# aanna0701/face-recognition-pytorch

Measured on AMD Instinct MI355X. Metric: train imgs/sec IR-50-layout ResNet50 + ArcFace/PartialFC head, 112x112, higher is better.
Workload: dtype bf16

## Files before the change

### face-recognition-pytorch_amd/frhip/csrc/misc.hip

```cpp
#include <stdarg.h>
#include <stdio.h>
#include <atomic>
#include "common.h"
#include "frhip.h"

namespace frhip {

static thread_local char g_err[512] = "";

void set_error(const char* fmt, ...) {
    va_list ap;
    va_start(ap, fmt);
    vsnprintf(g_err, sizeof(g_err), fmt, ap);
    va_end(ap);
}

int check_launch(const char* what) {
    hipError_t e = hipGetLastError();
    if (e != hipSuccess) {
        set_error("%s: launch failed: %s", what, hipGetErrorString(e));
        return FRHIP_ELAUNCH;
    }
    return FRHIP_OK;
}

int set_dynamic_lds(const void* fn, int bytes, const char* who) {
    constexpr int SLOTS = 256;
    static std::atomic<const void*> fns[SLOTS];
    static std::atomic<uint64_t> devs[SLOTS];
    int dev = 0;
    if (hipGetDevice(&dev) != hipSuccess) { (void)hipGetLastError(); dev = -1; }
    const uint64_t bit = (dev >= 0 && dev < 64) ? 1ull << dev : 0;
    int slot = -1;
    const size_t h = (size_t)(((uintptr_t)fn >> 4) * 0x9E3779B97F4A7C15ull >> 32);
    for (int i = 0; i < SLOTS && slot < 0; ++i) {
        const int s = (int)((h + i) % SLOTS);
        const void* cur = nullptr;
        if (fns[s].compare_exchange_strong(cur, fn) || cur == fn) slot = s;
    }
    if (slot >= 0 && bit && (devs[slot].load() & bit)) return FRHIP_OK;
    if (hipFuncSetAttribute(fn, hipFuncAttributeMaxDynamicSharedMemorySize, bytes) != hipSuccess) {
        set_error("%s: cannot raise dynamic LDS to %d bytes", who, bytes);
        return FRHIP_ELAUNCH;
    }
    if (slot >= 0) devs[slot].fetch_or(bit);
    return FRHIP_OK;
}

int device_cu_count() {
    static std::atomic<int> cus[16];
    int dev = 0;
    if (hipGetDevice(&dev) != hipSuccess || dev < 0 || dev >= 16) { (void)hipGetLastError(); return 256; }
    int v = cus[dev].load();
    if (!v) {
        if (hipDeviceGetAttribute(&v, hipDeviceAttributeMultiprocessorCount, dev) != hipSuccess || v <= 0) v = 256;
        cus[dev].store(v);
    }
    return v;
}

template <typename T>
__global__ void pack_wt_kernel(const float* __restrict__ w, T* __restrict__ wt, int K, int RS, int C) {
    __shared__ float tile[32][33];
    const int rs = blockIdx.z, c0 = blockIdx.x * 32, k0 = blockIdx.y * 32;
    for (int j = threadIdx.y; j < 32; j += blockDim.y) {
        const int k = k0 + j, c = c0 + threadIdx.x;
        tile[j][threadIdx.x] = (k < K && c < C) ? w[((size_t)k * RS + rs) * C + c] : 0.f;
    }
    __syncthreads();
    for (int j = threadIdx.y; j < 32; j += blockDim.y) {
        const int c = c0 + j, k = k0 + threadIdx.x;
        if (c < C && k < K) wt[((size_t)c * RS + rs) * K + k] = from_f32<T>(tile[threadIdx.x][j]);
    }
}

template <typename T>
__global__ void prep_weights_kernel(const frhip_wprep* __restrict__ tab, int ntensors) {
    __shared__ float tile[32][33];
    int lo = 0, hi = ntensors - 1;
    while (lo < hi) {
        const int mid = (lo + hi + 1) >> 1;
        if (tab[mid].tile_begin <= (int)blockIdx.x) lo = mid; else hi = mid - 1;
    }
    const frhip_wprep e = tab[lo];
    const int K = e.k, RS = e.rs, C = e.c;
    const int ct = (C + 31) >> 5, kt = (K + 31) >> 5;
    int t = (int)blockIdx.x - e.tile_begin;
    const int cti = t % ct; t /= ct;
    const int kti = t % kt; const int rs = t / kt;
    const int c0 = cti * 32, k0 = kti * 32;
    const float* __restrict__ w = e.w;
    T* __restrict__ wc = reinterpret_cast<T*>(e.wc);
    T* __restrict__ wt = reinterpret_cast<T*>(e.wt);
    for (int j = threadIdx.y; j < 32; j += blockDim.y) {
        const int k = k0 + j, c = c0 + threadIdx.x;
        float v = 0.f;
        if (k < K && c < C) {
            const size_t idx = ((size_t)k * RS + rs) * C + c;
            v = w[idx];
            if (wc) wc[idx] = from_f32<T>(v);
        }
        tile[j][threadIdx.x] = v;
    }
    __syncthreads();
    if (wt)
        for (int j = threadIdx.y; j < 32; j += blockDim.y) {
            const int c = c0 + j, k = k0 + threadIdx.x;
            if (c < C && k < K) wt[((size_t)c * RS + rs) * K + k] = from_f32<T>(tile[threadIdx.x][j]);
        }
}

template <typename TI, typename TO>
__global__ void transpose2d_kernel(const TI* __restrict__ in, TO* __restrict__ out, int rows, int cols, int ld_out) {
    __shared__ float tile[32][33];
    const int c0 = blockIdx.x * 32, r0 = blockIdx.y * 32;
    for (int j = threadIdx.y; j < 32; j += blockDim.y) {
        const int r = r0 + j, c = c0 + threadIdx.x;
        tile[j][threadIdx.x] = (r < rows && c < cols) ? to_f32<TI>(in[(size_t)r * cols + c]) : 0.f;
    }
    __syncthreads();
    for (int j = threadIdx.y; j < 32; j += blockDim.y) {
        const int c = c0 + j, r = r0 + threadIdx.x;
        if (c < cols && r < ld_out) out[(size_t)c * ld_out + r] = from_f32<TO>(tile[threadIdx.x][j]);
    }
}

template <typename T>
__global__ void pack_stem_kernel(const float* __restrict__ w, T* __restrict__ wp, int K, int kin, int kp) {
    const int i = blockIdx.x * blockDim.x + threadIdx.x;
    if (i >= K * kp) return;
    const int k = i / kp, j = i - k * kp;
    wp[i] = from_f32<T>(j < kin ? w[k * kin + j] : 0.f);
}
__global__ void unpack_stem_grad_kernel(const float* __restrict__ dwp, float* __restrict__ dw, int K, int kin, int kp) {
    const int i = blockIdx.x * blockDim.x + threadIdx.x;
    if (i >= K * kin) return;
    const int k = i / kin, j = i - k * kin;
    dw[i] += dwp[k * kp + j];
}

template <typename T>
__global__ __launch_bounds__(256) void fc_permute_kernel(const float* __restrict__ w, T* __restrict__ wp, int C, int HW) {
    extern __shared__ float sh[];
    const int n = blockIdx.x, c0 = blockIdx.y * 64;
    const size_t row = (size_t)n * C * HW;
    for (int i = threadIdx.x; i < 64 * HW; i += 256) sh[i] = w[row + (size_t)c0 * HW + i];
    __syncthreads();
    for (int i = threadIdx.x; i < 64 * HW; i += 256) {
        const int p = i / 64, c = i - p * 64;
        wp[row + (size_t)p * C + c0 + c] = from_f32<T>(sh[c * HW + p]);
    }
}
__global__ __launch_bounds__(256) void fc_unpermute_grad_kernel(const float* __restrict__ dwp, float* __restrict__ dw, int C, int HW) {
    extern __shared__ float sh[];
    const int n = blockIdx.x, c0 = blockIdx.y * 64;
    const size_t row = (size_t)n * C * HW;
    for (int i = threadIdx.x; i < 64 * HW; i += 256) {
        const int p = i / 64, c = i - p * 64;
        sh[i] = dwp[row + (size_t)p * C + c0 + c];
    }
    __syncthreads();
    for (int i = threadIdx.x; i < 64 * HW; i += 256) {
        const int c = i / HW, p = i - c * HW;
        dw[row + (size_t)c0 * HW + i] += sh[p * 64 + c];
    }
}

__global__ void gather_rows_kernel(const float* __restrict__ src, const int64_t* __restrict__ index,
                                   float* __restrict__ dst, int n, int D) {
    const int vpr = D / 4;
    for (size_t t = (size_t)blockIdx.x * blockDim.x + threadIdx.x; t < (size_t)n * vpr; t += (size_t)gridDim.x * blockDim.x) {
        const int i = (int)(t / vpr), v = (int)(t - (size_t)i * vpr);
        reinterpret_cast<f32x4_t*>(dst)[t] = reinterpret_cast<const f32x4_t*>(src)[(size_t)index[i] * vpr + v];
    }
}
__global__ void scatter_rows_kernel(const float* __restrict__ src, const int64_t* __restrict__ index,
                                    float* __restrict__ dst, int n, int D) {
    const int vpr = D / 4;
    for (size_t t = (size_t)blockIdx.x * blockDim.x + threadIdx.x; t < (size_t)n * vpr; t += (size_t)gridDim.x * blockDim.x) {
        const int i = (int)(t / vpr), v = (int)(t - (size_t)i * vpr);
        reinterpret_cast<f32x4_t*>(dst)[(size_t)index[i] * vpr + v] = reinterpret_cast<const f32x4_t*>(src)[t];
    }
}

}

using namespace frhip;

extern "C" const char* frhip_last_error(void) { return g_err; }
extern "C" int frhip_abi_version(void) { return 1; }

extern "C" int frhip_pack_wt(int dtype, const float* w, void* wt, int k, int rs, int c, hipStream_t stream) {
    return by_dtype(dtype, "frhip_pack_wt", [&](auto t) {
        typedef decltype(t) T;
        dim3 grid((c + 31) / 32, (k + 31) / 32, rs), block(32, 8);
        hipLaunchKernelGGL(pack_wt_kernel<T>, grid, block, 0, stream, w, (T*)wt, k, rs, c);
        return check_launch("frhip_pack_wt");
    });
}

extern "C" int frhip_prep_conv_weights(int dtype, const frhip_wprep* table, int ntensors, int ntiles, hipStream_t stream) {
    return by_dtype(dtype, "frhip_prep_conv_weights", [&](auto t) {
        typedef decltype(t) T;
        if (!table || ntensors < 1 || ntiles < 1) { set_error("frhip_prep_conv_weights: empty table"); return FRHIP_EINVAL; }
        dim3 block(32, 8);
        hipLaunchKernelGGL(prep_weights_kernel<T>, dim3(ntiles), block, 0, stream, table, ntensors);
        return check_launch("frhip_prep_conv_weights");
    });
}

extern "C" int frhip_transpose2d(int dtype_in, int dtype_out, const void* in, void* out, int rows, int cols, int ld_out, hipStream_t stream) {
    if (ld_out < rows) { set_error("frhip_transpose2d: ld_out %d < rows %d", ld_out, rows); return FRHIP_EINVAL; }
    dim3 grid((cols + 31) / 32, (ld_out + 31) / 32), block(32, 8);
    const int key = dtype_in * 2 + dtype_out;
    switch (key) {
        case 0: hipLaunchKernelGGL((transpose2d_kernel<bf16_t, bf16_t>), grid, block, 0, stream, (const bf16_t*)in, (bf16_t*)out, rows, cols, ld_out); break;
        case 1: hipLaunchKernelGGL((transpose2d_kernel<bf16_t, float>), grid, block, 0, stream, (const bf16_t*)in, (float*)out, rows, cols, ld_out); break;
        case 2: hipLaunchKernelGGL((transpose2d_kernel<float, bf16_t>), grid, block, 0, stream, (const float*)in, (bf16_t*)out, rows, cols, ld_out); break;
        case 3: hipLaunchKernelGGL((transpose2d_kernel<float, float>), grid, block, 0, stream, (const float*)in, (float*)out, rows, cols, ld_out); break;
        default: set_error("frhip_transpose2d: bad dtypes"); return FRHIP_EINVAL;
    }
    return check_launch("frhip_transpose2d");
}

extern "C" int frhip_pack_stem(int dtype, const float* w, void* wp, int k, int kin, int kp, hipStream_t stream) {
    return by_dtype(dtype, "frhip_pack_stem", [&](auto t) {
        typedef decltype(t) T;
        const int n = k * kp;
        hipLaunchKernelGGL(pack_stem_kernel<T>, dim3((n + 255) / 256), dim3(256), 0, stream, w, (T*)wp, k, kin, kp);
        return check_launch("frhip_pack_stem");
    });
}

extern "C" int frhip_unpack_stem_grad(const float* dwp, float* dw, int k, int kin, int kp, hipStream_t stream) {
    const int n = k * kin;
    hipLaunchKernelGGL(unpack_stem_grad_kernel, dim3((n + 255) / 256), dim3(256), 0, stream, dwp, dw, k, kin, kp);
    return check_launch("frhip_unpack_stem_grad");
}

extern "C" int frhip_fc_permute(int dtype, const float* w, void* wp, int nout, int c, int hw, hipStream_t stream) {
    return by_dtype(dtype, "frhip_fc_permute", [&](auto t) {
        typedef decltype(t) T;
        if (c % 64) { set_error("frhip_fc_permute: channels must be a multiple of 64"); return FRHIP_EINVAL; }
        dim3 grid(nout, c / 64);
        const int lds = 64 * hw * 4;
        hipLaunchKernelGGL(fc_permute_kernel<T>, grid, dim3(256), lds, stream, w, (T*)wp, c, hw);
        return check_launch("frhip_fc_permute");
    });
}

extern "C" int frhip_fc_unpermute_grad(const float* dwp, float* dw, int nout, int c, int hw, hipStream_t stream) {
    if (c % 64) { set_error("frhip_fc_unpermute_grad: channels must be a multiple of 64"); return FRHIP_EINVAL; }
    hipLaunchKernelGGL(fc_unpermute_grad_kernel, dim3(nout, c / 64), dim3(256), 64 * hw * 4, stream, dwp, dw, c, hw);
    return check_launch("frhip_fc_unpermute_grad");
}

extern "C" int frhip_gather_rows(const float* src, const int64_t* index, float* dst, int n, int d, hipStream_t stream) {
    if (d % 4) { set_error("frhip_gather_rows: row length must be a multiple of 4"); return FRHIP_EINVAL; }
    if (n == 0) return FRHIP_OK;
// ... 23 lines not shown
```

### face-recognition-pytorch_amd/frhip/csrc/stem_algebra.hip

```cpp
#include "common.h"
#include "frhip.h"

namespace frhip {

constexpr int SG_ROWS = 8;
constexpr int SG_ROLES = 8;
constexpr int SG_VALS = 81;
constexpr int SG_OUT = 7 * SG_VALS;

template <typename T>
__global__ __launch_bounds__(256) void stem_gram_kernel(const float* __restrict__ x, float* __restrict__ partial, int B, int H, int W) {
    extern __shared__ __attribute__((aligned(16))) char smem[];
    float* xs = reinterpret_cast<float*>(smem);
    const int XR = SG_ROWS + 2, XC = W + 2;
    const int role = threadIdx.x & 7, pl = threadIdx.x >> 3;
    const int ca_ = role < 3 ? 0 : (role < 5 ? 1 : 2);
    const int cb_ = role < 3 ? role : (role < 5 ? role - 2 : 2);
    float acc[SG_VALS];
#pragma unroll
    for (int i = 0; i < SG_VALS; ++i) acc[i] = 0.f;
    const int bands = (H + SG_ROWS - 1) / SG_ROWS;
    for (int tile = blockIdx.x; tile < B * bands; tile += gridDim.x) {
        const int n = tile / bands, h0 = (tile - n * bands) * SG_ROWS;
        const float* ximg = x + (size_t)n * 3 * H * W;
        __syncthreads();
        for (int idx = threadIdx.x; idx < 3 * XR * XC; idx += 256) {
            const int cc = idx % XC, rest = idx / XC, rr = rest % XR, ci = rest / XR;
            const int h = h0 - 1 + rr, w = cc - 1;
            const float v = ((unsigned)h < (unsigned)H && (unsigned)w < (unsigned)W) ? ximg[((size_t)ci * H + h) * W + w] : 0.f;
            xs[idx] = to_f32<T>(from_f32<T>(v));
        }
        __syncthreads();
        const int rows = min(SG_ROWS, H - h0);
        for (int p = pl; p < rows * W; p += 32) {
            const int py = p / W, px = p - py * W;
            const float* base = xs + py * XC + px;
            if (role < 6) {
                float va[9], vb[9];
#pragma unroll
                for (int a = 0; a < 9; ++a) {
                    va[a] = base[(ca_ * XR + a / 3) * XC + a % 3];
                    vb[a] = base[(cb_ * XR + a / 3) * XC + a % 3];
                }
#pragma unroll
                for (int a = 0; a < 9; ++a)
#pragma unroll
                    for (int b = 0; b < 9; ++b) acc[a * 9 + b] = fmaf(va[a], vb[b], acc[a * 9 + b]);
            } else if (role == 6) {
#pragma unroll
                for (int c = 0; c < 3; ++c)
#pragma unroll
                    for (int a = 0; a < 9; ++a) acc[c * 9 + a] += base[(c * XR + a / 3) * XC + a % 3];
            }
        }
    }
    __syncthreads();
    float* red = reinterpret_cast<float*>(smem);
    const int lane = lane_id(), wave = wave_id();
#pragma unroll
    for (int i = 0; i < SG_VALS; ++i) {
        float v = acc[i];
        v = lane_sum_bit3(v); v = lane_sum_bit4(v); v = lane_sum_bit5(v);
        if (lane < 8) red[(wave * 8 + lane) * SG_VALS + i] = v;
    }
    __syncthreads();
    for (int o = threadIdx.x; o < SG_OUT; o += 256)
        partial[(size_t)blockIdx.x * SG_OUT + o] = red[o] + red[8 * SG_VALS + o] + red[16 * SG_VALS + o] + red[24 * SG_VALS + o];
}

__global__ __launch_bounds__(256) void stem_gram_fold_kernel(const float* __restrict__ partial, int nparts, float* __restrict__ blk) {
    __shared__ float red[3][SG_VALS];
    const int o = threadIdx.x % SG_VALS, part = threadIdx.x / SG_VALS;
    if (part < 3) {
        float a = 0.f;
        for (int p = part; p < nparts; p += 3) a += partial[(size_t)p * SG_OUT + blockIdx.x * SG_VALS + o];
        red[part][o] = a;
    }
    __syncthreads();
    if (threadIdx.x < SG_VALS) blk[blockIdx.x * SG_VALS + o] = red[0][o] + red[1][o] + red[2][o];
}

__global__ __launch_bounds__(256) void stem_gram_assemble_kernel(const float* __restrict__ blk, float* __restrict__ gram) {
    for (int o = threadIdx.x; o < 27 * 27 + 27; o += 256) {
        if (o < 729) {
            const int j = o / 27, j2 = o - j * 27;
// ... 183 lines not shown
```

### face-recognition-pytorch_amd/frhip/csrc/stem_fused.hip

```cpp
#include "common.h"
#include "tr_frag.h"
#include "frhip.h"

namespace frhip {

constexpr int SF_PH = 4, SF_PW = 28;
constexpr int SF_RH = 2 * SF_PH + 1, SF_RW = 2 * SF_PW + 1;

template <typename T>
struct StemConv {
    static constexpr int EPL = 16 / (int)sizeof(T);
    static constexpr int RUNS = 32 / (4 * EPL);
    typedef typename Mma<T>::Frag Frag;
    Frag wf[RUNS][4];
    int koff[RUNS][EPL];
    const T* xs;
    int XR, XC;

    __device__ __forceinline__ void init(const T* __restrict__ wp, const T* xs_, int XR_, int XC_) {
        xs = xs_; XR = XR_; XC = XC_;
        const int lane = lane_id(), i = lane & 15, g = lane >> 4;
#pragma unroll
        for (int r = 0; r < RUNS; ++r) {
#pragma unroll
            for (int t = 0; t < 4; ++t)
                wf[r][t] = *reinterpret_cast<const Frag*>(wp + (t * 16 + i) * 32 + r * 4 * EPL + g * EPL);
#pragma unroll
            for (int e = 0; e < EPL; ++e) {
                const int k = r * 4 * EPL + g * EPL + e;
                const int tap = k / 3, ci = k - tap * 3, fr = tap / 3, fs = tap - fr * 3;
                koff[r][e] = k < 27 ? (ci * XR + fr) * XC + fs : 0;
            }
        }
    }
    __device__ __forceinline__ void stage(T* xs_w, const float* __restrict__ ximg, int h_org, int w_org, int H, int W) const {
        const int total = 3 * XR * XC;
        for (int idx = threadIdx.x; idx < total; idx += blockDim.x) {
            const int cc = idx % XC, rest = idx / XC;
            const int rr = rest % XR, ci = rest / XR;
            const int h = h_org + rr, w = w_org + cc;
            const float v = ((unsigned)h < (unsigned)H && (unsigned)w < (unsigned)W) ? ximg[((size_t)ci * H + h) * W + w] : 0.f;
            xs_w[idx] = from_f32<T>(v);
        }
    }
    __device__ __forceinline__ void gather(int hl, int wl, bool live, Frag (&b)[RUNS]) const {
        const int base = live ? hl * XC + wl : 0;
#pragma unroll
        for (int r = 0; r < RUNS; ++r) {
            Vec16<T> v;
#pragma unroll
            for (int e = 0; e < EPL; ++e) v.v[e] = xs[base + koff[r][e]];
            b[r] = v.v;
        }
    }
    __device__ __forceinline__ void conv(const Frag (&b)[RUNS], f32x4_t (&acc)[4]) const {
#pragma unroll
        for (int t = 0; t < 4; ++t) {
            acc[t] = f32x4_t{0.f, 0.f, 0.f, 0.f};
#pragma unroll
            for (int r = 0; r < RUNS; ++r) Mma<T>::run(wf[r][t], b[r], acc[t]);
        }
    }
};

__device__ __forceinline__ int sf_chan(int t, int reg) { return t * 16 + 4 * (lane_id() >> 4) + reg; }

__device__ __forceinline__ float sf_sum16(float v) { return lane_sum_row16(v); }

template <typename T>
__global__ __launch_bounds__(256) void stem_stats_kernel(const float* __restrict__ x, const T* __restrict__ wp,
                                                         float* __restrict__ partial, int B, int H, int W) {
    extern __shared__ __attribute__((aligned(16))) char smem[];
    T* xs = reinterpret_cast<T*>(smem);
    const int XR = 10, XC = W + 2;
    StemConv<T> sc;
    sc.init(wp, xs, XR, XC);
    const int lane = lane_id(), wave = wave_id(), i = lane & 15;
    const int bands = (H + 7) / 8;
    float s1[4][4], s2[4][4];
#pragma unroll
    for (int t = 0; t < 4; ++t)
#pragma unroll
        for (int r = 0; r < 4; ++r) { s1[t][r] = 0.f; s2[t][r] = 0.f; }
    for (int tile = blockIdx.x; tile < B * bands; tile += gridDim.x) {
        const int n = tile / bands, h0 = (tile - n * bands) * 8;
        __syncthreads();
        sc.stage(xs, x + (size_t)n * 3 * H * W, h0 - 1, -1, H, W);
        __syncthreads();
        for (int rr = 0; rr < 2; ++rr) {
            const int hl = wave * 2 + rr;
            if (h0 + hl >= H) break;
            for (int w0 = 0; w0 < W; w0 += 16) {
                const int w = w0 + i;
                typename StemConv<T>::Frag b[StemConv<T>::RUNS];
                f32x4_t acc[4];
                sc.gather(hl, w, w < W, b);
                sc.conv(b, acc);
#pragma unroll
                for (int t = 0; t < 4; ++t)
#pragma unroll
                    for (int r = 0; r < 4; ++r) { const float y = w < W ? acc[t][r] : 0.f; s1[t][r] += y; s2[t][r] += y * y; }
            }
        }
    }
    __syncthreads();
    float (*red)[2][64] = reinterpret_cast<float (*)[2][64]>(smem);
#pragma unroll
    for (int t = 0; t < 4; ++t)
#pragma unroll
        for (int r = 0; r < 4; ++r) {
            const float a = sf_sum16(s1[t][r]), b2 = sf_sum16(s2[t][r]);
            if (i == 0) { red[wave][0][sf_chan(t, r)] = a; red[wave][1][sf_chan(t, r)] = b2; }
        }
    __syncthreads();
    if (threadIdx.x < 128) {
        const int st = threadIdx.x >> 6, c = threadIdx.x & 63;
        partial[((size_t)blockIdx.x * 2 + st) * 64 + c] = red[0][st][c] + red[1][st][c] + red[2][st][c] + red[3][st][c];
    }
}

template <typename T>
__global__ __launch_bounds__(256) void stem_fwd_kernel(const float* __restrict__ x, const T* __restrict__ wp,
                                                       const float* __restrict__ scale, const float* __restrict__ shift,
                                                       T* __restrict__ pooled, uint8_t* __restrict__ argmax, int B, int H, int W) {
    constexpr int EPV = 16 / (int)sizeof(T), VPR = 64 / EPV;
    constexpr int PITCH = 64 * (int)sizeof(T) + 16;
    extern __shared__ __attribute__((aligned(16))) char smem[];
    constexpr int XR = SF_RH + 2, XC = SF_RW + 2;
    T* xs = reinterpret_cast<T*>(smem + SF_RH * SF_RW * PITCH);
    StemConv<T> sc;
    sc.init(wp, xs, XR, XC);
    const int lane = lane_id(), wave = wave_id(), i = lane & 15, g = lane >> 4;
    const int Hp = (H - 1) / 2 + 1, Wp = (W - 1) / 2 + 1;
    const int tw = (Wp + SF_PW - 1) / SF_PW, th = (Hp + SF_PH - 1) / SF_PH;
    int tile = blockIdx.x;
    const int n = tile / (tw * th); tile -= n * tw * th;
    const int ph0 = (tile / tw) * SF_PH, pw0 = (tile % tw) * SF_PW;
    sc.stage(xs, x + (size_t)n * 3 * H * W, 2 * ph0 - 2, 2 * pw0 - 2, H, W);
    __syncthreads();
    float sc_[4][4], sh_[4][4];
#pragma unroll
    for (int t = 0; t < 4; ++t)
#pragma unroll
        for (int r = 0; r < 4; ++r) { sc_[t][r] = scale[sf_chan(t, r)]; sh_[t][r] = shift[sf_chan(t, r)]; }
    for (int it = wave; it * 16 < SF_RH * SF_RW; it += 4) {
        const int rp = it * 16 + i;
        const int rr = rp / SF_RW, rc = rp - rr * SF_RW;
        const int h = 2 * ph0 - 1 + rr, w = 2 * pw0 - 1 + rc;
        const bool inside = rp < SF_RH * SF_RW && (unsigned)h < (unsigned)H && (unsigned)w < (unsigned)W;
        typename StemConv<T>::Frag b[StemConv<T>::RUNS];
        f32x4_t acc[4];
        sc.gather(rr, rc, rp < SF_RH * SF_RW, b);
        sc.conv(b, acc);
        if (rp < SF_RH * SF_RW) {
#pragma unroll
            for (int t = 0; t < 4; ++t) {
                T* dst = reinterpret_cast<T*>(smem + rp * PITCH) + t * 16 + 4 * g;
#pragma unroll
                for (int r = 0; r < 4; ++r) {
                    const float a = fmaxf(acc[t][r] * sc_[t][r] + sh_[t][r], 0.f);
                    dst[r] = from_f32<T>(inside ? a : -INFINITY);
                }
            }
        }
    }
    __syncthreads();
    for (int task = threadIdx.x; task < SF_PH * SF_PW * VPR; task += 256) {
        const int cv = task % VPR, pp = task / VPR;
        const int pl = pp / SF_PW, pc = pp - pl * SF_PW;
        const int ph = ph0 + pl, pw = pw0 + pc;
        if (ph >= Hp || pw >= Wp) continue;
        float best[EPV]; int bi[EPV];
#pragma unroll
        for (int e = 0; e < EPV; ++e) { best[e] = -INFINITY; bi[e] = 0; }
#pragma unroll
        for (int r = 0; r < 3; ++r)
#pragma unroll
            for (int s = 0; s < 3; ++s) {
                const Vec16<T> v = *reinterpret_cast<const Vec16<T>*>(smem + ((2 * pl + r) * SF_RW + 2 * pc + s) * PITCH + cv * 16);
#pragma unroll
                for (int e = 0; e < EPV; ++e) {
                    const float a = v.get(e);
                    if (a > best[e]) { best[e] = a; bi[e] = r * 3 + s; }
                }
            }
        const size_t o = ((((size_t)n * Hp + ph) * Wp + pw) * VPR + cv) * EPV;
        Vec16<T> ov;
#pragma unroll
        for (int e = 0; e < EPV; ++e) ov.set(e, best[e]);
        *reinterpret_cast<Vec16<T>*>(pooled + o) = ov;
        if constexpr (EPV == 8) {
            uint64_t pk = 0;
#pragma unroll
            for (int e = 0; e < 8; ++e) pk |= (uint64_t)(uint32_t)bi[e] << (8 * e);
            *reinterpret_cast<uint64_t*>(argmax + o) = pk;
        } else {
            uint32_t pk = 0;
#pragma unroll
            for (int e = 0; e < 4; ++e) pk |= (uint32_t)bi[e] << (8 * e);
            *reinterpret_cast<uint32_t*>(argmax + o) = pk;
        }
    }
}

template <typename T, bool WGRAD>
__global__ __launch_bounds__(256, 2) void stem_bwd_kernel(const float* __restrict__ x, const T* __restrict__ wp,
                                                       const T* __restrict__ dpool, const uint8_t* __restrict__ argmax,
                                                       const float* __restrict__ p0, const float* __restrict__ p1,
                                                       const float* __restrict__ p2, const float* __restrict__ scale,
                                                       const float* __restrict__ shift, float* __restrict__ outbuf,
                                                       int B, int H, int W) {
    constexpr int EPL = StemConv<T>::EPL, RUNS = StemConv<T>::RUNS;
    constexpr int TH = SF_PH + 1, TW = SF_PW + 1;
    constexpr int DROW = 64 * (int)sizeof(T) + 16;
    constexpr int AROW = 64 + 16;
    constexpr int DY_RB = 64 * (int)sizeof(T), COL_RB = 128;
    constexpr int KR = TnFrag<T, 128>::KROWS;
    constexpr int SUB = KR / 16;
    extern __shared__ __attribute__((aligned(16))) char smem[];
    char* s_dp = smem;
    uint8_t* s_arg = reinterpret_cast<uint8_t*>(smem + TH * TW * DROW);
    char* s_wg = smem + TH * TW * (DROW + AROW);
    constexpr int XR = 2 * SF_PH + 2, XC = 2 * SF_PW + 2;
    T* xs = reinterpret_cast<T*>(s_wg + (WGRAD ? 4 * KR * (DY_RB + COL_RB) : 0) + 5 * 64 * 4);
    StemConv<T> sc;
    sc.init(wp, xs, XR, XC);
    const int lane = lane_id(), wave = wave_id(), i = lane & 15, g = lane >> 4;
    char* my_dy = s_wg + wave * KR * (DY_RB + COL_RB);
    char* my_col = my_dy + KR * DY_RB;
    const int Hp = (H - 1) / 2 + 1, Wp = (W - 1) / 2 + 1;
    const int tw = (Wp + SF_PW - 1) / SF_PW, th = (Hp + SF_PH - 1) / SF_PH;
    float* s_const = reinterpret_cast<float*>(s_wg + (WGRAD ? 4 * KR * (DY_RB + COL_RB) : 0));
    for (int v = threadIdx.x; v < 64; v += 256) {
        s_const[v] = scale[v]; s_const[64 + v] = shift[v];
        if (WGRAD) { s_const[128 + v] = p0[v]; s_const[192 + v] = p1[v]; s_const[256 + v] = p2[v]; }
    }
    auto cvec = [&](int which, int t) { return *reinterpret_cast<const f32x4_t*>(s_const + which * 64 + t * 16 + 4 * g); };
    float s1[4][4], s2[4][4];
    f32x4_t dw[4][2];
#pragma unroll
    for (int t = 0; t < 4; ++t) {
#pragma unroll
        for (int r = 0; r < 4; ++r) { s1[t][r] = 0.f; s2[t][r] = 0.f; }
        dw[t][0] = f32x4_t{0.f, 0.f, 0.f, 0.f}; dw[t][1] = dw[t][0];
    }
    if (WGRAD && sizeof(T) == 2) {
        for (int v = lane; v < KR * COL_RB / 16; v += 64) *reinterpret_cast<f32x4_t*>(my_col + v * 16) = f32x4_t{0.f, 0.f, 0.f, 0.f};
    }

    for (int tile = blockIdx.x; tile < B * th * tw; tile += gridDim.x) {
        int rem = tile;
        const int n = rem / (tw * th); rem -= n * tw * th;
        const int ph0 = (rem / tw) * SF_PH, pw0 = (rem % tw) * SF_PW;
// ... 545 lines not shown
    for (int v = threadIdx.x; v < 9 * 64; v += 256) {
        const int tap = v >> 6, k = v & 63;
        const T* wr = wp + (size_t)k * kp + tap * 3;
        s_w[v] = f32x4_t{(float)wr[0], (float)wr[1], (float)wr[2], 0.f};
    }
    __syncthreads();
    const int Ho = (H - 1) / 2 + 1, Wo = (W - 1) / 2 + 1;
    const size_t total = (size_t)B * Ho * Wo;
    for (size_t q = (size_t)blockIdx.x * 256 + threadIdx.x; q < total; q += (size_t)gridDim.x * 256) {
        const int b = (int)(q % Wo);
        const size_t rest = q / Wo;
        const int a = (int)(rest % Ho), n = (int)(rest / Ho);
        const bool r1 = a + 1 < Ho, c1 = b + 1 < Wo;
        const T* row00 = dy0 + (((size_t)n * Ho + a) * Wo + b) * 64;
        const T* row01 = c1 ? row00 + 64 : row00;
        const T* row10 = r1 ? row00 + (size_t)Wo * 64 : row00;
        const T* row11 = r1 && c1 ? row10 + 64 : row00;
        f32x4_t p00 = {0.f, 0.f, 0.f, 0.f}, p01 = p00, p10 = p00, p11 = p00;
#pragma unroll 2
        for (int kc = 0; kc < VPT; ++kc) {
            const Vec16<T> v00 = *reinterpret_cast<const Vec16<T>*>(row00 + kc * EPV);
            const Vec16<T> v01 = *reinterpret_cast<const Vec16<T>*>(row01 + kc * EPV);
            const Vec16<T> v10 = *reinterpret_cast<const Vec16<T>*>(row10 + kc * EPV);
            const Vec16<T> v11 = *reinterpret_cast<const Vec16<T>*>(row11 + kc * EPV);
#pragma unroll
            for (int e = 0; e < EPV; ++e) {
                const int k = kc * EPV + e;
                const float q00 = v00.get(e), q01 = c1 ? v01.get(e) : 0.f, q10 = r1 ? v10.get(e) : 0.f, q11 = r1 && c1 ? v11.get(e) : 0.f;
                const f32x4_t w00 = s_w[0 * 64 + k], w01 = s_w[1 * 64 + k], w02 = s_w[2 * 64 + k], w10 = s_w[3 * 64 + k], w11 = s_w[4 * 64 + k],
                              w12 = s_w[5 * 64 + k], w20 = s_w[6 * 64 + k], w21 = s_w[7 * 64 + k], w22 = s_w[8 * 64 + k];
                p00 += w11 * q00;
                p01 += w10 * q01 + w12 * q00;
                p10 += w01 * q10 + w21 * q00;
                p11 += w00 * q11 + w02 * q10 + w20 * q01 + w22 * q00;
            }
        }
        const size_t plane = (size_t)H * W, o = ((size_t)n * 3 * H + 2 * a) * W + 2 * b;
        const bool hr = 2 * a + 1 < H, wc = 2 * b + 1 < W;
#pragma unroll
        for (int c = 0; c < 3; ++c) {
            float* d = dx + o + c * plane;
            d[0] = p00[c];
            if (wc) d[1] = p01[c];
            if (hr) d[W] = p10[c];
            if (hr && wc) d[W + 1] = p11[c];
        }
    }
}

}

using namespace frhip;

extern "C" int frhip_stem_blocks(int b, int h, int w) {
    const int t = sf_tiles(b, h, w);
    return t < 1024 ? t : 1024;
}

static bool sf_ok(int dtype, int b, int h, int w, const char* who) {
    if ((dtype != FRHIP_DT_BF16 && dtype != FRHIP_DT_F32) || b <= 0 || h <= 0 || w <= 0 ||
        3LL * b * h * w > 0x7fffffffLL) {
        set_error("%s: unsupported dtype / shape (dtype=%d b=%d h=%d w=%d)", who, dtype, b, h, w);
        return false;
    }
    return true;
}

extern "C" int frhip_stem_stats(int dtype, const float* x, const void* wp, int b, int h, int w, float* partial,
                                hipStream_t stream) {
    return by_dtype(dtype, "frhip_stem_stats", [&](auto t) {
        typedef decltype(t) T;
        if (!sf_ok(dtype, b, h, w, "frhip_stem_stats")) return FRHIP_EINVAL;
        const int blocks = frhip_stem_blocks(b, h, w);
        int lds = 3 * 10 * (w + 2) * (int)sizeof(T);
        if (lds < 4 * 2 * 64 * 4) lds = 4 * 2 * 64 * 4;
        if (lds > 64 * 1024) { set_error("frhip_stem_stats: image too wide (%d)", w); return FRHIP_EINVAL; }
        hipLaunchKernelGGL(stem_stats_kernel<T>, dim3(blocks), dim3(256), lds, stream, x, (const T*)wp, partial, b, h, w);
        return check_launch("frhip_stem_stats");
    });
}

template <typename T>
static int sf_fwd(const float* x, const void* wp, const float* scale, const float* shift, void* pooled, uint8_t* argmax,
                  int b, int h, int w, hipStream_t stream) {
    const int lds = SF_RH * SF_RW * (64 * (int)sizeof(T) + 16) + 3 * (SF_RH + 2) * (SF_RW + 2) * (int)sizeof(T);
    auto kern = stem_fwd_kernel<T>;
    if (set_dynamic_lds(reinterpret_cast<const void*>(kern), lds, "frhip_stem_fwd")) return FRHIP_ELAUNCH;
    hipLaunchKernelGGL(kern, dim3(sf_tiles(b, h, w)), dim3(256), lds, stream, x, (const T*)wp, scale, shift, (T*)pooled, argmax, b, h, w);
    return check_launch("frhip_stem_fwd");
}

extern "C" int frhip_stem_fwd(int dtype, const float* x, const void* wp, const float* scale, const float* shift,
                              void* pooled, uint8_t* argmax, int b, int h, int w, hipStream_t stream) {
    return by_dtype(dtype, "frhip_stem_fwd", [&](auto t) {
        if (!sf_ok(dtype, b, h, w, "frhip_stem_fwd")) return FRHIP_EINVAL;
        return sf_fwd<decltype(t)>(x, wp, scale, shift, pooled, argmax, b, h, w, stream);
    });
}

template <typename T, bool WGRAD>
static int sf_bwd(const float* x, const void* wp, const void* dpool, const uint8_t* argmax, const float* p0, const float* p1,
                  const float* p2, const float* scale, const float* shift, float* outbuf, int b, int h, int w,
                  hipStream_t stream, const char* who) {
    constexpr int KR = sizeof(T) == 2 ? 32 : 16;
    const int tile_bytes = (SF_PH + 1) * (SF_PW + 1) * (64 * (int)sizeof(T) + 16 + 80) +
                           (WGRAD ? 4 * KR * (64 * (int)sizeof(T) + 128) : 0) + 5 * 64 * 4 +
                           3 * (2 * SF_PH + 2) * (2 * SF_PW + 2) * (int)sizeof(T);
    const int red_bytes = WGRAD ? 4 * 64 * 32 * 4 : 4 * 2 * 64 * 4;
    const int lds = tile_bytes > red_bytes ? tile_bytes : red_bytes;
    auto kern = stem_bwd_kernel<T, WGRAD>;
    if (set_dynamic_lds(reinterpret_cast<const void*>(kern), lds, who)) return FRHIP_ELAUNCH;
    hipLaunchKernelGGL(kern, dim3(frhip_stem_blocks(b, h, w)), dim3(256), lds, stream, x, (const T*)wp, (const T*)dpool, argmax,
                       p0, p1, p2, scale, shift, outbuf, b, h, w);
    return check_launch(who);
}

template <bool WGRAD>
static int sf_bwd2(const float* x, const void* wp, const void* dpool, const uint8_t* argmax, const float* p0, const float* p1,
                   const float* p2, const float* scale, const float* shift, float* outbuf, int b, int h, int w,
                   hipStream_t stream, const char* who) {
    const int lds = WGRAD ? SB_LDS_WGRAD : SB_LDS_REDUCE;
    static_assert(SB_LDS_WGRAD >= SB_WAVES * 64 * 32 * 4 && SB_LDS_WGRAD <= 160 * 1024, "LDS budget");
    auto kern = stem_bwd2_kernel<WGRAD>;
    if (set_dynamic_lds(reinterpret_cast<const void*>(kern), lds, who)) return FRHIP_ELAUNCH;
    hipLaunchKernelGGL(kern, dim3(frhip_stem_blocks(b, h, w)), dim3(SB_THREADS), lds, stream, x, (const bf16_t*)wp,
                       (const bf16_t*)dpool, argmax, p0, p1, p2, scale, shift, outbuf, b, h, w);
    return check_launch(who);
}

static int g_stem_scatter = 1;

extern "C" int frhip_stem_bwd_reduce(int dtype, const float* x, const void* wp, const void* dpool, const uint8_t* argmax,
                                     const float* mean, const float* invstd, const float* scale, const float* shift,
                                     int b, int h, int w, float* partial, hipStream_t stream) {
    return by_dtype(dtype, "frhip_stem_bwd_reduce", [&](auto t) {
        if (!sf_ok(dtype, b, h, w, "frhip_stem_bwd_reduce")) return FRHIP_EINVAL;
        if (dtype == FRHIP_DT_BF16 && g_stem_scatter)
            return sf_bwd2<false>(x, wp, dpool, argmax, mean, invstd, nullptr, scale, shift, partial, b, h, w, stream, "frhip_stem_bwd_reduce");
        return sf_bwd<decltype(t), false>(x, wp, dpool, argmax, mean, invstd, nullptr, scale, shift, partial, b, h, w, stream,
                                          "frhip_stem_bwd_reduce");
    });
// ... 59 lines not shown
```

Measured before the change: 23020.

## Prefetch next stem tiles into registers and batch weight-prep tiles per block

The stem gram, stats and forward kernels now load the next tile's input band into registers while the current tile is computed, replacing the sync-load-sync staging. The forward kernel becomes persistent with a grid capped at 1024 blocks. The weight-prep kernel processes runs of 8 tiles per block with register prefetch and paired stores, and the stats kernel gains an occupancy hint. The goal is to hide global load latency and cut launch and block overhead, at the cost of more registers per thread and fewer blocks in flight.

New measurement: 23120 (median of 6 runs). No clear change (+0.5%).

```diff
diff --git a/face-recognition-pytorch_amd/frhip/csrc/misc.hip b/face-recognition-pytorch_amd/frhip/csrc/misc.hip
--- a/face-recognition-pytorch_amd/frhip/csrc/misc.hip
+++ b/face-recognition-pytorch_amd/frhip/csrc/misc.hip
@@ -1,6 +1,7 @@
 #include <stdarg.h>
 #include <stdio.h>
 #include <atomic>
+#include <type_traits>
 #include "common.h"
 #include "frhip.h"
 
@@ -74,40 +75,91 @@
     }
 }
 
+constexpr int WP_RUN = 8;
+
+struct WprepTile {
+    const float* w; void* wc; void* wt;
+    int K, RS, C, rs, c0, k0;
+};
+
+__device__ __forceinline__ WprepTile wprep_tile(const frhip_wprep& e, int tile) {
+    WprepTile d;
+    d.w = e.w; d.wc = e.wc; d.wt = e.wt; d.K = e.k; d.RS = e.rs; d.C = e.c;
+    const int ct = (e.c + 31) >> 5, kt = (e.k + 31) >> 5;
+    int t = tile - e.tile_begin;
+    d.c0 = (t % ct) * 32; t /= ct;
+    d.k0 = (t % kt) * 32; d.rs = t / kt;
+    return d;
+}
+
+__device__ __forceinline__ void wprep_load(const WprepTile& d, float (&v)[4]) {
+#pragma unroll
+    for (int q = 0; q < 4; ++q) {
+        const int k = d.k0 + (int)threadIdx.y + 8 * q, c = d.c0 + (int)threadIdx.x;
+        v[q] = 0.f;
+        if (k < d.K && c < d.C) v[q] = d.w[((size_t)k * d.RS + d.rs) * d.C + c];
+    }
+}
+
+template <typename T, bool TR>
+__device__ __forceinline__ void wprep_store(T* __restrict__ out, const float (*tile)[33], int r0, int rows, int x0, int cols,
+                                            size_t row_stride, size_t base) {
+    typedef typename std::conditional<sizeof(T) == 2, uint32_t, uint64_t>::type Pair;
+    const int tid = (int)threadIdx.y * 32 + (int)threadIdx.x;
+    const int xx = (tid & 15) * 2;
+    const bool paired = ((row_stride | base) & 1) == 0 && (reinterpret_cast<uintptr_t>(out) & (2 * sizeof(T) - 1)) == 0;
+#pragma unroll
+    for (int q = 0; q < 2; ++q) {
+        const int r = (tid >> 4) + 16 * q;
+        if (r0 + r >= rows || x0 + xx >= cols) continue;
+        const float a = TR ? tile[xx][r] : tile[r][xx], b = TR ? tile[xx + 1][r] : tile[r][xx + 1];
+        T* dst = out + base + (size_t)(r0 + r) * row_stride + x0 + xx;
+        if (paired && x0 + xx + 1 < cols) {
+            const T two[2] = {from_f32<T>(a), from_f32<T>(b)};
+            Pair pr;
+            __builtin_memcpy(&pr, two, sizeof(pr));
+            *reinterpret_cast<Pair*>(dst) = pr;
+        } else {
+            dst[0] = from_f32<T>(a);
+            if (x0 + xx + 1 < cols) dst[1] = from_f32<T>(b);
+        }
+    }
+}
+
 template <typename T>
-__global__ void prep_weights_kernel(const frhip_wprep* __restrict__ tab, int ntensors) {
+__global__ __launch_bounds__(256) void prep_weights_kernel(const frhip_wprep* __restrict__ tab, int ntensors, int ntiles) {
     __shared__ float tile[32][33];
+    const int first = (int)blockIdx.x * WP_RUN, last = min(first + WP_RUN, ntiles);
     int lo = 0, hi = ntensors - 1;
     while (lo < hi) {
         const int mid = (lo + hi + 1) >> 1;
-        if (tab[mid].tile_begin <= (int)blockIdx.x) lo = mid; else hi = mid - 1;
-    }
-    const frhip_wprep e = tab[lo];
-    const int K = e.k, RS = e.rs, C = e.c;
-    const int ct = (C + 31) >> 5, kt = (K + 31) >> 5;
-    int t = (int)blockIdx.x - e.tile_begin;
-    const int cti = t % ct; t /= ct;
-    const int kti = t % kt; const int rs = t / kt;
-    const int c0 = cti * 32, k0 = kti * 32;
-    const float* __restrict__ w = e.w;
-    T* __restrict__ wc = reinterpret_cast<T*>(e.wc);
-    T* __restrict__ wt = reinterpret_cast<T*>(e.wt);
-    for (int j = threadIdx.y; j < 32; j += blockDim.y) {
-        const int k = k0 + j, c = c0 + threadIdx.x;
-        float v = 0.f;
-        if (k < K && c < C) {
-            const size_t idx = ((size_t)k * RS + rs) * C + c;
-            v = w[idx];
-            if (wc) wc[idx] = from_f32<T>(v);
+        if (tab[mid].tile_begin <= first) lo = mid; else hi = mid - 1;
+    }
+    int next_begin = lo + 1 < ntensors ? tab[lo + 1].tile_begin : ntiles;
+    frhip_wprep e = tab[lo];
+    WprepTile cur = wprep_tile(e, first);
+    float v[4];
+    wprep_load(cur, v);
+    for (int t = first; t < last; ++t) {
+        __syncthreads();
+#pragma unroll
+        for (int q = 0; q < 4; ++q) tile[(int)threadIdx.y + 8 * q][threadIdx.x] = v[q];
+        __syncthreads();
+        WprepTile nxt = cur;
+        if (t + 1 < last) {
+            if (t + 1 >= next_begin) {
+                ++lo;
+                e = tab[lo];
+                next_begin = lo + 1 < ntensors ? tab[lo + 1].tile_begin : ntiles;
+            }
+            nxt = wprep_tile(e, t + 1);
+            wprep_load(nxt, v);
         }
-        tile[j][threadIdx.x] = v;
-    }
-    __syncthreads();
-    if (wt)
-        for (int j = threadIdx.y; j < 32; j += blockDim.y) {
-            const int c = c0 + j, k = k0 + threadIdx.x;
-            if (c < C && k < K) wt[((size_t)c * RS + rs) * K + k] = from_f32<T>(tile[threadIdx.x][j]);
-        }
+        const size_t rsK = (size_t)cur.RS * cur.K, rsC = (size_t)cur.RS * cur.C;
+        if (cur.wc) wprep_store<T, false>(reinterpret_cast<T*>(cur.wc), tile, cur.k0, cur.K, cur.c0, cur.C, rsC, (size_t)cur.rs * cur.C);
+        if (cur.wt) wprep_store<T, true>(reinterpret_cast<T*>(cur.wt), tile, cur.c0, cur.C, cur.k0, cur.K, rsK, (size_t)cur.rs * cur.K);
+        cur = nxt;
+    }
 }
 
 template <typename TI, typename TO>
@@ -204,7 +256,7 @@
         typedef decltype(t) T;
         if (!table || ntensors < 1 || ntiles < 1) { set_error("frhip_prep_conv_weights: empty table"); return FRHIP_EINVAL; }
         dim3 block(32, 8);
-        hipLaunchKernelGGL(prep_weights_kernel<T>, dim3(ntiles), block, 0, stream, table, ntensors);
+        hipLaunchKernelGGL(prep_weights_kernel<T>, dim3((ntiles + WP_RUN - 1) / WP_RUN), block, 0, stream, table, ntensors, ntiles);
         return check_launch("frhip_prep_conv_weights");
     });
 }
diff --git a/face-recognition-pytorch_amd/frhip/csrc/stem_algebra.hip b/face-recognition-pytorch_amd/frhip/csrc/stem_algebra.hip
--- a/face-recognition-pytorch_amd/frhip/csrc/stem_algebra.hip
+++ b/face-recognition-pytorch_amd/frhip/csrc/stem_algebra.hip
@@ -1,4 +1,5 @@
 #include "common.h"
+#include "stem_stage.h"
 #include "frhip.h"
 
 namespace frhip {
@@ -20,17 +21,23 @@
 #pragma unroll
     for (int i = 0; i < SG_VALS; ++i) acc[i] = 0.f;
     const int bands = (H + SG_ROWS - 1) / SG_ROWS;
-    for (int tile = blockIdx.x; tile < B * bands; tile += gridDim.x) {
+    float pre[StemBand<SG_ROWS + 2>::N];
+    auto cvt = [](float v) { return to_f32<T>(from_f32<T>(v)); };
+    const int ntiles = B * bands;
+    if ((int)blockIdx.x < ntiles) {
+        const int n = blockIdx.x / bands, h0 = (blockIdx.x - n * bands) * SG_ROWS;
+        stem_band_load<SG_ROWS + 2>(pre, x + (size_t)n * 3 * H * W, 0, h0 - 1, H, W);
+    }
+    for (int tile = blockIdx.x; tile < ntiles; tile += gridDim.x) {
         const int n = tile / bands, h0 = (tile - n * bands) * SG_ROWS;
-        const float* ximg = x + (size_t)n * 3 * H * W;
-        __syncthreads();
-        for (int idx = threadIdx.x; idx < 3 * XR * XC; idx += 256) {
-            const int cc = idx % XC, rest = idx / XC, rr = rest % XR, ci = rest / XR;
-            const int h = h0 - 1 + rr, w = cc - 1;
-            const float v = ((unsigned)h < (unsigned)H && (unsigned)w < (unsigned)W) ? ximg[((size_t)ci * H + h) * W + w] : 0.f;
-            xs[idx] = to_f32<T>(from_f32<T>(v));
-        }
-        __syncthreads();
+        __syncthreads();
+        stem_band_store<SG_ROWS + 2>(xs, pre, 0, XC, cvt);
+        stem_band_rest<SG_ROWS + 2>(xs, x + (size_t)n * 3 * H * W, h0 - 1, H, W, cvt);
+        __syncthreads();
+        if (tile + (int)gridDim.x < ntiles) {
+            const int nt = tile + gridDim.x, n2 = nt / bands, h2 = (nt - n2 * bands) * SG_ROWS;
+            stem_band_load<SG_ROWS + 2>(pre, x + (size_t)n2 * 3 * H * W, 0, h2 - 1, H, W);
+        }
         const int rows = min(SG_ROWS, H - h0);
         for (int p = pl; p < rows * W; p += 32) {
             const int py = p / W, px = p - py * W;
diff --git a/face-recognition-pytorch_amd/frhip/csrc/stem_fused.hip b/face-recognition-pytorch_amd/frhip/csrc/stem_fused.hip
--- a/face-recognition-pytorch_amd/frhip/csrc/stem_fused.hip
+++ b/face-recognition-pytorch_amd/frhip/csrc/stem_fused.hip
@@ -1,5 +1,6 @@
 #include "common.h"
 #include "tr_frag.h"
+#include "stem_stage.h"
 #include "frhip.h"
 
 namespace frhip {
@@ -43,6 +44,14 @@
             xs_w[idx] = from_f32<T>(v);
         }
     }
+    template <int N>
+    __device__ __forceinline__ void load(float (&r)[N], const float* __restrict__ ximg, int h_org, int w_org, int H, int W) const {
+        stem_window_load<N>(r, ximg, 0, XR, XC, h_org, w_org, H, W);
+    }
+    template <int N>
+    __device__ __forceinline__ void store(T* xs_w, const float (&r)[N]) const {
+        stem_window_store<N>(xs_w, r, 0, 3 * XR * XC, [](float v) { return from_f32<T>(v); });
+    }
     __device__ __forceinline__ void gather(int hl, int wl, bool live, Frag (&b)[RUNS]) const {
         const int base = live ? hl * XC + wl : 0;
 #pragma unroll
@@ -68,7 +77,7 @@
 __device__ __forceinline__ float sf_sum16(float v) { return lane_sum_row16(v); }
 
 template <typename T>
-__global__ __launch_bounds__(256) void stem_stats_kernel(const float* __restrict__ x, const T* __restrict__ wp,
+__global__ __launch_bounds__(256, sizeof(T) == 2 ? 4 : 2) void stem_stats_kernel(const float* __restrict__ x, const T* __restrict__ wp,
                                                          float* __restrict__ partial, int B, int H, int W) {
     extern __shared__ __attribute__((aligned(16))) char smem[];
     T* xs = reinterpret_cast<T*>(smem);
@@ -82,11 +91,24 @@
     for (int t = 0; t < 4; ++t)
 #pragma unroll
         for (int r = 0; r < 4; ++r) { s1[t][r] = 0.f; s2[t][r] = 0.f; }
-    for (int tile = blockIdx.x; tile < B * bands; tile += gridDim.x) {
+    float pre[StemBand<10>::N];
+    auto cvt = [](float v) { return from_f32<T>(v); };
+    const int ntiles = B * bands;
+    if ((int)blockIdx.x < ntiles) {
+        const int n = blockIdx.x / bands, h0 = (blockIdx.x - n * bands) * 8;
+        stem_band_load<10>(pre, x + (size_t)n * 3 * H * W, 0, h0 - 1, H, W);
+    }
+    stem_loads_landed();
+    for (int tile = blockIdx.x; tile < ntiles; tile += gridDim.x) {
         const int n = tile / bands, h0 = (tile - n * bands) * 8;
         __syncthreads();
-        sc.stage(xs, x + (size_t)n * 3 * H * W, h0 - 1, -1, H, W);
-        __syncthreads();
+        stem_band_store<10>(xs, pre, 0, XC, cvt);
+        stem_band_rest<10>(xs, x + (size_t)n * 3 * H * W, h0 - 1, H, W, cvt);
+        __syncthreads();
+        if (tile + (int)gridDim.x < ntiles) {
+            const int nt = tile + gridDim.x, n2 = nt / bands, h2 = (nt - n2 * bands) * 8;
+            stem_band_load<10>(pre, x + (size_t)n2 * 3 * H * W, 0, h2 - 1, H, W);
+        }
         for (int rr = 0; rr < 2; ++rr) {
             const int hl = wave * 2 + rr;
             if (h0 + hl >= H) break;
@@ -127,78 +149,98 @@
     constexpr int PITCH = 64 * (int)sizeof(T) + 16;
     extern __shared__ __attribute__((aligned(16))) char smem[];
     constexpr int XR = SF_RH + 2, XC = SF_RW + 2;
+    constexpr int PRE = (3 * XR * XC + 255) / 256;
     T* xs = reinterpret_cast<T*>(smem + SF_RH * SF_RW * PITCH);
     StemConv<T> sc;
     sc.init(wp, xs, XR, XC);
     const int lane = lane_id(), wave = wave_id(), i = lane & 15, g = lane >> 4;
     const int Hp = (H - 1) / 2 + 1, Wp = (W - 1) / 2 + 1;
     const int tw = (Wp + SF_PW - 1) / SF_PW, th = (Hp + SF_PH - 1) / SF_PH;
-    int tile = blockIdx.x;
-    const int n = tile / (tw * th); tile -= n * tw * th;
-    const int ph0 = (tile / tw) * SF_PH, pw0 = (tile % tw) * SF_PW;
-    sc.stage(xs, x + (size_t)n * 3 * H * W, 2 * ph0 - 2, 2 * pw0 - 2, H, W);
-    __syncthreads();
+    const int ntiles = B * th * tw;
+    float pre[PRE];
+    if ((int)blockIdx.x < ntiles) {
+        int rem = blockIdx.x;
+        const int n = rem / (tw * th); rem -= n * tw * th;
+        sc.template load<PRE>(pre, x + (size_t)n * 3 * H * W, 2 * ((rem / tw) * SF_PH) - 2, 2 * ((rem % tw) * SF_PW) - 2, H, W);
+    }
     float sc_[4][4], sh_[4][4];
 #pragma unroll
     for (int t = 0; t < 4; ++t)
 #pragma unroll
         for (int r = 0; r < 4; ++r) { sc_[t][r] = scale[sf_chan(t, r)]; sh_[t][r] = shift[sf_chan(t, r)]; }
-    for (int it = wave; it * 16 < SF_RH * SF_RW; it += 4) {
-        const int rp = it * 16 + i;
-        const int rr = rp / SF_RW, rc = rp - rr * SF_RW;
-        const int h = 2 * ph0 - 1 + rr, w = 2 * pw0 - 1 + rc;
-        const bool inside = rp < SF_RH * SF_RW && (unsigned)h < (unsigned)H && (unsigned)w < (unsigned)W;
-        typename StemConv<T>::Frag b[StemConv<T>::RUNS];
-        f32x4_t acc[4];
-        sc.gather(rr, rc, rp < SF_RH * SF_RW, b);
-        sc.conv(b, acc);
-        if (rp < SF_RH * SF_RW) {
-#pragma unroll
-            for (int t = 0; t < 4; ++t) {
-                T* dst = reinterpret_cast<T*>(smem + rp * PITCH) + t * 16 + 4 * g;
-#pragma unroll
-                for (int r = 0; r < 4; ++r) {
-                    const float a = fmaxf(acc[t][r] * sc_[t][r] + sh_[t][r], 0.f);
-                    dst[r] = from_f32<T>(inside ? a : -INFINITY);
-                }
-            }
-        }
-    }
-    __syncthreads();
-    for (int task = threadIdx.x; task < SF_PH * SF_PW * VPR; task += 256) {
-        const int cv = task % VPR, pp = task / VPR;
-        const int pl = pp / SF_PW, pc = pp - pl * SF_PW;
-        const int ph = ph0 + pl, pw = pw0 + pc;
-        if (ph >= Hp || pw >= Wp) continue;
-        float best[EPV]; int bi[EPV];
-#pragma unroll
-        for (int e = 0; e < EPV; ++e) { best[e] = -INFINITY; bi[e] = 0; }
-#pragma unroll
-        for (int r = 0; r < 3; ++r)
-#pragma unroll
-            for (int s = 0; s < 3; ++s) {
-                const Vec16<T> v = *reinterpret_cast<const Vec16<T>*>(smem + ((2 * pl + r) * SF_RW + 2 * pc + s) * PITCH + cv * 16);
-#pragma unroll
-                for (int e = 0; e < EPV; ++e) {
-                    const float a = v.get(e);
-                    if (a > best[e]) { best[e] = a; bi[e] = r * 3 + s; }
-                }
-            }
-        const size_t o = ((((size_t)n * Hp + ph) * Wp + pw) * VPR + cv) * EPV;
-        Vec16<T> ov;
-#pragma unroll
-        for (int e = 0; e < EPV; ++e) ov.set(e, best[e]);
-        *reinterpret_cast<Vec16<T>*>(pooled + o) = ov;
-        if constexpr (EPV == 8) {
-            uint64_t pk = 0;
-#pragma unroll
-            for (int e = 0; e < 8; ++e) pk |= (uint64_t)(uint32_t)bi[e] << (8 * e);
-            *reinterpret_cast<uint64_t*>(argmax + o) = pk;
-        } else {
-            uint32_t pk = 0;
-#pragma unroll
-            for (int e = 0; e < 4; ++e) pk |= (uint32_t)bi[e] << (8 * e);
-            *reinterpret_cast<uint32_t*>(argmax + o) = pk;
+    stem_loads_landed();
+#pragma unroll
+    for (int t = 0; t < 4; ++t)
+#pragma unroll
+        for (int r = 0; r < 4; ++r) { stem_value_landed(sc_[t][r]); stem_value_landed(sh_[t][r]); }
+    for (int tile = blockIdx.x; tile < ntiles; tile += gridDim.x) {
+        int rem = tile;
+        const int n = rem / (tw * th); rem -= n * tw * th;
+        const int ph0 = (rem / tw) * SF_PH, pw0 = (rem % tw) * SF_PW;
+        sc.template store<PRE>(xs, pre);
+        __syncthreads();
+        if (tile + (int)gridDim.x < ntiles) {
+            int r2 = tile + gridDim.x;
+            const int n2 = r2 / (tw * th); r2 -= n2 * tw * th;
+            sc.template load<PRE>(pre, x + (size_t)n2 * 3 * H * W, 2 * ((r2 / tw) * SF_PH) - 2, 2 * ((r2 % tw) * SF_PW) - 2, H, W);
+        }
+        for (int it = wave; it * 16 < SF_RH * SF_RW; it += 4) {
+            const int rp = it * 16 + i;
+            const int rr = rp / SF_RW, rc = rp - rr * SF_RW;
+            const int h = 2 * ph0 - 1 + rr, w = 2 * pw0 - 1 + rc;
+            const bool inside = rp < SF_RH * SF_RW && (unsigned)h < (unsigned)H && (unsigned)w < (unsigned)W;
+            typename StemConv<T>::Frag b[StemConv<T>::RUNS];
+            f32x4_t acc[4];
+            sc.gather(rr, rc, rp < SF_RH * SF_RW, b);
+            sc.conv(b, acc);
+            if (rp < SF_RH * SF_RW) {
+#pragma unroll
+                for (int t = 0; t < 4; ++t) {
+                    T* dst = reinterpret_cast<T*>(smem + rp * PITCH) + t * 16 + 4 * g;
+#pragma unroll
+                    for (int r = 0; r < 4; ++r) {
+                        const float a = fmaxf(acc[t][r] * sc_[t][r] + sh_[t][r], 0.f);
+                        dst[r] = from_f32<T>(inside ? a : -INFINITY);
+                    }
+                }
+            }
+        }
+        __syncthreads();
+        for (int task = threadIdx.x; task < SF_PH * SF_PW * VPR; task += 256) {
+            const int cv = task % VPR, pp = task / VPR;
+            const int pl = pp / SF_PW, pc = pp - pl * SF_PW;
+            const int ph = ph0 + pl, pw = pw0 + pc;
+            if (ph >= Hp || pw >= Wp) continue;
+            float best[EPV]; int bi[EPV];
+#pragma unroll
+            for (int e = 0; e < EPV; ++e) { best[e] = -INFINITY; bi[e] = 0; }
+#pragma unroll
+            for (int r = 0; r < 3; ++r)
+#pragma unroll
+                for (int s = 0; s < 3; ++s) {
+                    const Vec16<T> v = *reinterpret_cast<const Vec16<T>*>(smem + ((2 * pl + r) * SF_RW + 2 * pc + s) * PITCH + cv * 16);
+#pragma unroll
+                    for (int e = 0; e < EPV; ++e) {
+                        const float a = v.get(e);
+                        if (a > best[e]) { best[e] = a; bi[e] = r * 3 + s; }
+                    }
+                }
+            const size_t o = ((((size_t)n * Hp + ph) * Wp + pw) * VPR + cv) * EPV;
+            Vec16<T> ov;
+#pragma unroll
+            for (int e = 0; e < EPV; ++e) ov.set(e, best[e]);
+            *reinterpret_cast<Vec16<T>*>(pooled + o) = ov;
+            if constexpr (EPV == 8) {
+                uint64_t pk = 0;
+#pragma unroll
+                for (int e = 0; e < 8; ++e) pk |= (uint64_t)(uint32_t)bi[e] << (8 * e);
+                *reinterpret_cast<uint64_t*>(argmax + o) = pk;
+            } else {
+                uint32_t pk = 0;
+#pragma unroll
+                for (int e = 0; e < 4; ++e) pk |= (uint32_t)bi[e] << (8 * e);
+                *reinterpret_cast<uint32_t*>(argmax + o) = pk;
+            }
         }
     }
 }
@@ -850,6 +892,8 @@
 
 using namespace frhip;
 
+constexpr int SF_FWD_MAX_BLOCKS = 1024;
+
 extern "C" int frhip_stem_blocks(int b, int h, int w) {
     const int t = sf_tiles(b, h, w);
     return t < 1024 ? t : 1024;
@@ -884,7 +928,8 @@
     const int lds = SF_RH * SF_RW * (64 * (int)sizeof(T) + 16) + 3 * (SF_RH + 2) * (SF_RW + 2) * (int)sizeof(T);
     auto kern = stem_fwd_kernel<T>;
     if (set_dynamic_lds(reinterpret_cast<const void*>(kern), lds, "frhip_stem_fwd")) return FRHIP_ELAUNCH;
-    hipLaunchKernelGGL(kern, dim3(sf_tiles(b, h, w)), dim3(256), lds, stream, x, (const T*)wp, scale, shift, (T*)pooled, argmax, b, h, w);
+    const int tiles = sf_tiles(b, h, w), blocks = tiles < SF_FWD_MAX_BLOCKS ? tiles : SF_FWD_MAX_BLOCKS;
+    hipLaunchKernelGGL(kern, dim3(blocks), dim3(256), lds, stream, x, (const T*)wp, scale, shift, (T*)pooled, argmax, b, h, w);
     return check_launch("frhip_stem_fwd");
 }
 
diff --git a/face-recognition-pytorch_amd/frhip/csrc/stem_stage.h b/face-recognition-pytorch_amd/frhip/csrc/stem_stage.h
--- /dev/null
+++ b/face-recognition-pytorch_amd/frhip/csrc/stem_stage.h
@@ -0,0 +1,76 @@
+#pragma once
+#include "common.h"
+
+namespace frhip {
+
+template <int N>
+__device__ __forceinline__ void stem_window_load(float (&r)[N], const float* __restrict__ ximg, int first, int XR, int XC,
+                                                 int h_org, int w_org, int H, int W) {
+    const int total = 3 * XR * XC;
+#pragma unroll
+    for (int j = 0; j < N; ++j) {
+        const int idx = first + (int)threadIdx.x + j * (int)blockDim.x;
+        const int cc = idx % XC, rest = idx / XC;
+        const int rr = rest % XR, ci = rest / XR;
+        const int h = h_org + rr, w = w_org + cc;
+        float v = 0.f;
+        if (idx < total && (unsigned)h < (unsigned)H && (unsigned)w < (unsigned)W) v = ximg[((size_t)ci * H + h) * W + w];
+        r[j] = v;
+    }
+}
+
+template <int N, typename E, typename CVT>
+__device__ __forceinline__ void stem_window_store(E* xs_w, const float (&r)[N], int first, int total, CVT cvt) {
+#pragma unroll
+    for (int j = 0; j < N; ++j) {
+        const int idx = first + (int)threadIdx.x + j * (int)blockDim.x;
+        if (idx < total) xs_w[idx] = cvt(r[j]);
+    }
+}
+
+__device__ __forceinline__ void stem_loads_landed() { __builtin_amdgcn_s_waitcnt(0x0F70); }
+__device__ __forceinline__ void stem_value_landed(float& v) { asm volatile("" : "+v"(v)); }
+
+constexpr int STEM_BAND_COLS = 128;
+template <int XR> struct StemBand {
+    static_assert(XR % 2 == 0, "two row groups");
+    static constexpr int N = 3 * XR / 2;
+};
+
+template <int XR>
+__device__ __forceinline__ void stem_band_load(float (&r)[StemBand<XR>::N], const float* __restrict__ ximg, int cb, int h_org, int H, int W) {
+    const int cc = cb * STEM_BAND_COLS + ((int)threadIdx.x & (STEM_BAND_COLS - 1)), rg = (int)threadIdx.x >> 7;
+    const bool colok = (unsigned)(cc - 1) < (unsigned)W;
+    const uint32_t voff = (uint32_t)(rg * W + cc) * 4u;
+#pragma unroll
+    for (int ci = 0; ci < 3; ++ci)
+#pragma unroll
+        for (int jr = 0; jr < XR / 2; ++jr) {
+            const int h = h_org + rg + 2 * jr;
+            const char* sbase = reinterpret_cast<const char*>(ximg) + ((long long)(ci * H + h_org + 2 * jr) * W - 1) * 4;
+            float v = 0.f;
+            if (colok && (unsigned)h < (unsigned)H) v = *reinterpret_cast<const float*>(sbase + voff);
+            r[ci * (XR / 2) + jr] = v;
+        }
+}
+
+template <int XR, typename E, typename CVT>
+__device__ __forceinline__ void stem_band_store(E* xs_w, const float (&r)[StemBand<XR>::N], int cb, int XC, CVT cvt) {
+    const int cc = cb * STEM_BAND_COLS + ((int)threadIdx.x & (STEM_BAND_COLS - 1)), rg = (int)threadIdx.x >> 7;
+    if (cc >= XC) return;
+#pragma unroll
+    for (int ci = 0; ci < 3; ++ci)
+#pragma unroll
+        for (int jr = 0; jr < XR / 2; ++jr) xs_w[(ci * XR + rg + 2 * jr) * XC + cc] = cvt(r[ci * (XR / 2) + jr]);
+}
+
+template <int XR, typename E, typename CVT>
+__device__ __forceinline__ void stem_band_rest(E* xs_w, const float* __restrict__ ximg, int h_org, int H, int W, CVT cvt) {
+    for (int cb = 1; cb * STEM_BAND_COLS < W + 2; ++cb) {
+        float r[StemBand<XR>::N];
+        stem_band_load<XR>(r, ximg, cb, h_org, H, W);
+        stem_band_store<XR>(xs_w, r, cb, W + 2, cvt);
+    }
+}
+
+}
```
